# lukashermann/hulc

Hardware: AMD Instinct MI355X
Metric: trajectory-windows/sec (seq_len=32, bs=64/GPU) (higher is better)
Workload: dtype bf16; 1 GPU; HULC training step, vision goal only (use_clip_auxiliary_loss=false), B=64 windows/GPU, seq_len=32, 200x200 static + 84x84 gripper fp32 NCHW frames, fwd+loss+bwd+Adam, dropout 0.1; global_batch=64, seq_len=32, parallelism=dp1

## Files before the change

### hulc_amd/csrc/engine_backward.inc

```
    struct Bucket { int64_t lo, hi; };
    Bucket group_range(const char* prefix) const {
        int64_t lo = numel, hi = 0;
        const std::string a(prefix);
        for (size_t i = 0; i < tab_order.size(); ++i) {
            const auto& kv = tab_order[i];
            if (kv.first.compare(0, a.size(), a) == 0) { lo = std::min(lo, kv.second.off); hi = std::max(hi, i + 1 < tab_order.size() ? tab_order[i + 1].second.off : numel); }
        }
        if (hi <= lo) return Bucket{0, 0};
        return Bucket{lo, std::min<int64_t>(hi, numel)};
    }
    std::vector<std::pair<std::string, Ref>> tab_order;
    std::vector<Bucket> bucket_plan() const {
        std::vector<Bucket> v;
        const Bucket dec = group_range("action_decoder.");
        v.push_back(Bucket{dec.lo, numel});
        v.push_back(group_range("plan_proposal."));
        v.push_back(group_range("plan_recognition."));
        const Bucket vg = group_range("visual_goal."), lg = group_range("language_goal.");
        v.push_back(Bucket{std::min(vg.lo, lg.lo), std::max(vg.hi, lg.hi)});
        v.push_back(group_range("perceptual_encoder."));
        return v;
    }
    int comm_buckets(int64_t* lo, int64_t* hi, int cap) override {
        if (!bound) { hulc_set_error("hulc_comm_buckets before hulc_bind_params"); return -1; }
// ... 215 lines not shown
            }
            }
            if (mlp) {
                lin_wgrad(dH1, H1, HID, SB, HID, HID, mlp2.dW, HID, mlp2.db);
                { EpiP ep = epi(dZ1, false); ep.mask = H1; lin_dgrad(dH1, SB, mlp2, ep, dense_out(HID)); }
                lin_wgrad(dZ1, H0, HID, SB, HID, HID, mlp1.dW, HID, mlp1.db);
                { EpiP ep = epi(dZ0, false); ep.mask = H0; lin_dgrad(dZ1, SB, mlp1, ep, dense_out(HID)); }
                const int mp = ldpad(SB);
                transpose_pair(dZ0, HID, tA, SB, HID, embg, DE, tB, SB, DE, mp, cs16 ? dbih0 : nullptr, nullptr);
                h0t_valid = false;
                { EpiP ep = epi(dwih0 + dec_plan, true); ep.accumulate = 1; gemm(dense<T>(tA, HID, mp), dense<T>(tB, DE, mp), dense_out(KIN), ep, HID, DE, SB); }
            } else {
            rnn_bwd(dH1, H1, dZ1, whh1, B, S, 1, false, false, true);
            {
                const int mp = ldpad(SB);
                const bool fuse_cs = cs16;
                bool h0t_kept = false;
                if constexpr (std::is_same<T, h16_t>::value) {
                    if (!tB2) tB2 = alloc<T>(tcap);
                    if (tB2) { transpose_triple(dZ1, HID, tA, SB, HID, H1, HID, tB, SB, HID, H0, HID, tB2, SB, HID, mp, fuse_cs ? dbih1 : nullptr, fuse_cs ? dbhh1 : nullptr); h0t_kept = true; }
                }
                if (!h0t_kept)
                transpose_pair(dZ1, HID, tA, SB, HID, H1, HID, tB, SB, HID, mp, fuse_cs ? dbih1 : nullptr, fuse_cs ? dbhh1 : nullptr);
                h0t_valid = h0t_kept;
                if (S > 1) { EpiP ep = epi(whh1.dW, true); ep.accumulate = grad_first(whh1.dW) ? 0 : 1;
                  gemm(dense<T>(tA + B, HID, mp), dense<T>(tB, HID, mp), dense_out(HID), ep, HID, HID, (S - 1) * B); }
                if (!h0t_kept) cast_tr<T, T>(H0, HID, nullptr, 0, tB, mp, SB, HID);
                { EpiP ep = epi(wih1.dW, true); ep.accumulate = grad_first(wih1.dW) ? 0 : 1; gemm(dense<T>(tA, HID, mp), dense<T>(h0t_kept ? tB2 : tB, HID, mp), dense_out(HID), ep, HID, HID, SB); }
                if (!fuse_cs) colsum(dZ1, HID, SB, HID, dbih1, dbhh1);
            }
            { EpiP ep = epi(dH0, false); ep.out2 = dZ0 + lastBH; ep.out2_lo = lastBH; ep.out2_hi = lastBH + BH; ep.out2_mask = H0 + lastBH;
              gemm(dense<T>(dZ1, SB, HID), dense<T>(wih1.Wt, HID, HID), dense_out(HID), ep, SB, HID, HID); }
            rnn_bwd(dH0, H0, dZ0, whh0, B, S, 1, false, false, true);
            {
                const int mp = ldpad(SB);
                if (h0t_valid) {
                    transpose_pair(dZ0, HID, tA, SB, HID, embg, DE, tB, SB, DE, mp, cs16 ? dbih0 : nullptr, cs16 ? dbhh0 : nullptr);
                    if (S > 1) { EpiP ep = epi(whh0.dW, true); ep.accumulate = grad_first(whh0.dW) ? 0 : 1;
                      gemm(dense<T>(tA + B, HID, mp), dense<T>(tB2, HID, mp), dense_out(HID), ep, HID, HID, (S - 1) * B); }
                } else {
                transpose_pair(dZ0, HID, tA, SB, HID, H0, HID, tB, SB, HID, mp, cs16 ? dbih0 : nullptr, cs16 ? dbhh0 : nullptr);
                if (S > 1) { EpiP ep = epi(whh0.dW, true); ep.accumulate = grad_first(whh0.dW) ? 0 : 1;
                  gemm(dense<T>(tA + B, HID, mp), dense<T>(tB, HID, mp), dense_out(HID), ep, HID, HID, (S - 1) * B); }
                cast_tr<T, T>(embg, DE, nullptr, 0, tB, mp, SB, DE);
                }
                { EpiP ep = epi(dwih0 + dec_plan, true); ep.accumulate = 1; gemm(dense<T>(tA, HID, mp), dense<T>(tB, DE, mp), dense_out(KIN), ep, HID, DE, SB); }
            }
            }
            if (!bwd_skip_enc) { EpiP ep = epi(demb + (EMB - DE), true); ep.accumulate = 1;
              gemm(dense<T>(dZ0, SB, HID), dense<T>(wih0T + (long long)dec_plan * HID, DE, HID), dense_out_map(B, EMB, (long long)S * EMB), ep, SB, DE, HID); }
            hipLaunchKernelGGL((sum_over_t_kernel<T>), dim3(cdiv(BH, 256)), dim3(256), 0, st, dZ0, S, BH, dC);
            if constexpr (!std::is_same<T, h16_t>::value) colsum(dC, HID, B, HID, dbih0, dbhh0);
            else if (!cs16) colsum(dZ0, HID, SB, HID, dbih0, dbhh0);
            { EpiP ep = epi(dgoal, true); ep.accumulate = 1;
              gemm(dense<T>(dC, B, HID), dense<T>(wih0T + (long long)(dec_plan + DE) * HID, GOAL, HID), dense_out(GOAL), ep, B, GOAL, HID); }
            {
                const int mp = ldpad(B);
                transpose_pair(dC, HID, tA, B, HID, goal_t, GOAL, tB, B, GOAL, mp);
                EpiP ep = epi(dwih0 + dec_plan + DE, true); ep.accumulate = 1;
                gemm(dense<T>(tA, HID, mp), dense<T>(tB, GOAL, mp), dense_out(KIN), ep, HID, GOAL, B);
            }
            if (hulc) {
                { EpiP ep = epi(dplan, true); gemm(dense<T>(dC, B, HID), dense<T>(wih0T, PLAN, HID), dense_out(PLAN), ep, B, PLAN, HID); }
                launch_plan_scatter_grad<T>(st, plan_scatter_w4<T>(NCLS), dC, pidx, B, NCAT, NCLS, HID, KIN, dwih0, grads_fresh ? 1 : 0);
            }
            if (mcil) {
                { EpiP ep = epi(dplan, true); gemm(dense<T>(dC, B, HID), dense<T>(wih0T, dec_plan, HID), dense_out(dec_plan), ep, B, dec_plan, HID); }
                lin_wgrad(dC, plan_t, dec_plan, B, HID, dec_plan, dwih0, KIN, nullptr);
            }
        }
        const bool hold_buckets = hold_buckets_mode && mcil && !gru && ar_dtype >= 0 && persist_mode && !persist_under_comm && !(rp_probed && !rp_ok);
        if (!hold_buckets && bucket_ready(0)) return 1;
        if (hulc) {
            launch_st_softmax_bwd<T>(st, probs, dplan, dpr_kl, dpp_kl, B * NCAT, NCLS, dprl, dprl_t, dppl_t);
            DenseOut om = dense_out(EMB + GOAL);
            mlp_bwd(dppl_t, ppx, EMB + GOAL, B, pp, 5, ppa, dt_a, dt_a + (long long)B * HID, dppx, &om, 0);
            hipLaunchKernelGGL(pp_input_bwd_kernel, dim3(cdiv(B * (EMB + GOAL), 256)), dim3(256), 0, st, dppx, B, EMB, GOAL, demb, (long long)S * EMB, dgoal);
            if (bucket_ready(1)) return 1;
            if (wq_small(B)) wq_add(dprl_t, seqf_t, B, pr_fs);
            else lin_wgrad(dprl_t, seqf_t, FCH, B, PLAN, FCH, pr_fs.dW, FCH, pr_fs.db);
            { EpiP ep = epi(dseqf, true);
              if (have_dseq) ep.accumulate = 1;
              else { ep.out2 = dseq_t; ep.out2_lo = 0; ep.out2_hi = (long long)B * FCH; dseq_cast_done = true; }
              lin_dgrad(dprl_t, B, pr_fs, ep, dense_out(FCH)); }
            have_dseq = true;
        }
        if (mcil) {
            const int n = PLAN / 2;
            launch_normal_rsample_bwd<T>(st, dplan, plan_eps, pr_logits, dpr_kl, B, n, dprl_t);
            hipLaunchKernelGGL((cast_kernel<float, T>), dim3(cdiv(B * PLAN, 256)), dim3(256), 0, st, dpp_kl, dppl_t, (long long)B * PLAN);
            DenseOut om = dense_out(EMB + GOAL);
            mlp_bwd(dppl_t, ppx, EMB + GOAL, B, pp, 5, ppa, dt_a, dt_a + (long long)B * HID, dppx, &om, 0);
            hipLaunchKernelGGL(pp_input_bwd_kernel, dim3(cdiv(B * (EMB + GOAL), 256)), dim3(256), 0, st, dppx, B, EMB, GOAL, demb, (long long)S * EMB, dgoal);
            if (!hold_buckets && bucket_ready(1)) return 1;
            if (gru) bigru_bwd(dprl_t, B, S); else birnn_bwd(dprl_t, B, S);
            if (hold_buckets && (bucket_ready(0) || bucket_ready(1))) return 1;
        }
        if (have_dseq) {
            if (!dseq_cast_done) hipLaunchKernelGGL((cast_kernel<float, T>), dim3(cdiv(B * FCH, 256)), dim3(256), 0, st, dseqf, dseq_t, (long long)B * FCH);
            if (wq_small(B)) wq_add(dseq_t, xm, B, pr_fc);
            else lin_wgrad(dseq_t, xm, EMB, B, FCH, EMB, pr_fc.dW, EMB, pr_fc.db);
            { EpiP ep = epi(dxm, true); lin_dgrad(dseq_t, B, pr_fc, ep, dense_out(EMB)); }
            float* dx = dxa; float* dnext = dxb;
            if (!ln_bwd_can_bcast) hipLaunchKernelGGL(bcast_over_s_kernel, dim3(cdiv((long long)N * EMB, 256)), dim3(256), 0, st, dxm, B, S, EMB, dx);
            for (int l = 1; l >= 0; --l) {
                const bool bc = ln_bwd_can_bcast && l == 1;
                bool ffn_fused = false;
                if constexpr (std::is_same<T, h16_t>::value) ffn_fused = trf_on() && S <= 64;
                T *b_c = dt_c, *b_a = dt_a, *b_d = dt_c, *b_b = dt_b;
                bool defer_w = false;
                if constexpr (std::is_same<T, h16_t>::value) {
                    defer_w = ffn_fused;
                    if (defer_w) {
                        if (!trb_c[l]) { trb_c[l] = alloc<T>((int64_t)maxN * EMB); trb_a[l] = alloc<T>((int64_t)maxN * FF); trb_d[l] = alloc<T>((int64_t)maxN * EMB, l ? "tr_bd1" : "tr_bd0"); trb_b[l] = alloc<T>((int64_t)maxN * 3 * EMB, l ? "tr_bb1" : "tr_bb0"); }
                        b_c = trb_c[l]; b_a = trb_a[l]; b_d = trb_d[l]; b_b = trb_b[l];
                    }
// ... 41 lines not shown
                else lin_wgrad(b_d, ao[l], EMB, N, EMB, EMB, tr_out[l].dW, EMB, tr_out[l].db);
                { EpiP ep = epi(dt_a, false); lin_dgrad(b_d, N, tr_out[l], ep, dense_out(EMB)); }
                launch_attention_bwd<T>(st, attention_s64(S), qkv[l], Pat[l], dt_a, B, S, EMB, NH, b_b, dp, site_seed(1 + 4 * l));
                if (defer_w) wq_add(b_b, xt[l], N, tr_in[l]);
                else lin_wgrad(b_b, xt[l], EMB, N, 3 * EMB, EMB, tr_in[l].dW, EMB, tr_in[l].db);
                { EpiP ep = epi(dx, true); ep.res = dy_f; ep.res_f32 = 1; ep.res_ld = EMB; lin_dgrad(b_b, N, tr_in[l], ep, dense_out(EMB)); }
            }
            {
                const int bchunk = (std::is_same<T, float>::value || repro) ? B : 8;
                if (cdiv(B, bchunk) > 1) nd(ND_POS_EMB);
                hipLaunchKernelGGL(pr_input_bwd_kernel, dim3(cdiv(S * EMB, 256), cdiv(B, bchunk)), dim3(256), 0, st, dx, B, S, EMB, dp, site_seed(0), demb, dpos, bchunk);
            }
        }
        if (bucket_ready(1) || bucket_ready(2)) return 1;
        if (pair) {
            const int Bv = pairBv, Bl = B - pairBv;
            T* av[2] = {gl1, gl2};
            T* al[2] = {gl1 + (long long)Bv * HID, gl2 + (long long)Bv * HID};
            ln_bwd(dgoal, GOAL, gl3, GOAL, goal_st, ln_vg_g, Bv, GOAL, nullptr, 0, 0, dgl3_t, GOAL, d_ln_vg_g, d_ln_vg_b);
            DenseOut om = dense_out((long long)S * EMB);
            mlp_bwd(dgl3_t, emb + (long long)(S - 1) * EMB, (long long)S * EMB, Bv, vg, 3, av, dt_a, dt_a + (long long)B * HID, bwd_skip_enc ? nullptr : demb + (long long)(S - 1) * EMB, bwd_skip_enc ? nullptr : &om, bwd_skip_enc ? 0 : 1);
            ln_bwd(dgoal + Bv * GOAL, GOAL, gl3 + Bv * GOAL, GOAL, goal_st + 2 * Bv, ln_lg_g, Bl, GOAL, nullptr, 0, 0, dgl3_t + Bv * GOAL, GOAL, d_ln_lg_g, d_ln_lg_b);
            mlp_bwd(dgl3_t + Bv * GOAL, lang_t, LANG, Bl, lg, 3, al, dt_a, dt_a + (long long)B * HID, nullptr, nullptr, 0);
        } else {
            T* acts[2] = {gl1, gl2};
            if (b->is_lang) {
                ln_bwd(dgoal, GOAL, gl3, GOAL, goal_st, ln_lg_g, B, GOAL, nullptr, 0, 0, dgl3_t, GOAL, d_ln_lg_g, d_ln_lg_b);
                mlp_bwd(dgl3_t, lang_t, LANG, B, lg, 3, acts, dt_a, dt_a + (long long)B * HID, nullptr, nullptr, 0);
            } else {
                ln_bwd(dgoal, GOAL, gl3, GOAL, goal_st, ln_vg_g, B, GOAL, nullptr, 0, 0, dgl3_t, GOAL, d_ln_vg_g, d_ln_vg_b);
                DenseOut om = dense_out((long long)S * EMB);
                mlp_bwd(dgl3_t, emb + (long long)(S - 1) * EMB, (long long)S * EMB, B, vg, 3, acts, dt_a, dt_a + (long long)B * HID,
                        bwd_skip_enc ? nullptr : demb + (long long)(S - 1) * EMB, bwd_skip_enc ? nullptr : &om, bwd_skip_enc ? 0 : 1);
            }
        }
        }
        wq_flush();
        if (bucket_ready(3)) return 1;
        if (part == 0) {
            lazy_sweep(0, numel, st);
            if (hipGetLastError() != hipSuccess) { hulc_set_error("kernel launch failed in backward"); return 1; }
            bwd_stage = 1;
            return 0;
        }
        if (bwd_skip_enc) goto finish;
    encoders:
        {
            const Conv1Src src[2] = {conv1_src(*b, false), conv1_src(*b, true)}, src2[2] = {conv1_src(cur2, false), conv1_src(cur2, true)};
            const int Nenc = enc_frames(N);
            const bool tail_fused = enc_tail_fusable() && (!repro || enc_tail_bwd_room(Nenc));
            if (ragged()) launch_rows_reduce(st, demb, rg_lens(), rg_off(), B, S, EMB, demb_c);
            if (tail_fused) enc_tail_bwd_both(Nenc);
            enc_bwd_both(src, pair ? src2 : nullptr, Nenc, tail_fused);
            flush_unpacks();
        }
    finish:
        if (bucket_ready(4)) return 1;
        lazy_sweep(0, numel, st);
        if (hipGetLastError() != hipSuccess) { hulc_set_error("kernel launch failed in backward"); return 1; }
        have_fwd = false;
        bwd_stage = 0;
        grads_fresh = false;
        return 0;
    }
```

### hulc_amd/csrc/engine_encoders.inc

```
    ConvGeom geom(int Nf, int IH, int C, int K, int S) const {
        ConvGeom g; g.Nf = Nf; g.IH = g.IW = IH; g.C = C; g.KH = g.KW = K; g.S = S; g.OH = g.OW = (IH - K) / S + 1; return g;
    }
    Conv1Src conv1_src(const hulc_batch& b, bool gripper) const {
        Conv1Src s;
        s.X = gripper ? b.rgb_gripper : b.rgb_static;
        s.u8 = b.frames_u8 != 0;
        s.shift = s.u8 ? (gripper ? b.shift_gripper : b.shift_static) : nullptr;
        s.pad = gripper ? b.pad_gripper : b.pad_static;
        s.fold = (s.u8 && std::is_same<T, h16_t>::value && u8_fold_mode) ? 1 : 0;
        if (s.u8 && b.window_start) { s.wstart = reinterpret_cast<const long long*>(b.window_start); s.S = b.S; s.nstore = b.store_frames; }
        if (s.wstart && (b.window_len || b.window_len_host)) {
            const int set = &b == &cur2 ? 1 : 0;
            s.wstart = wl_frame[set]; s.S = 1;
            if (s.shift) s.shift = wl_shift[set][gripper ? 1 : 0];
        }
        return s;
    }
    static Conv1Src conv1_src_f32(const void* x) { return Conv1Src{x, nullptr, 0, 0}; }
    long long* wl_frame[2] = {nullptr, nullptr};
    int* wl_shift[2][2] = {{nullptr, nullptr}, {nullptr, nullptr}};
    int wl_alloc(int set) {
        if (!wl_frame[set]) {
            wl_frame[set] = alloc<long long>((int64_t)maxN); wl_shift[set][0] = alloc<int>((int64_t)maxN * 2); wl_shift[set][1] = alloc<int>((int64_t)maxN * 2);
            if (alloc_failed) { hulc_set_error("window_len: workspace allocation failed"); return 1; }
// ... 158 lines not shown
            const Stage S = stage(0, sn, Nf), G = stage(1, sn, Nf);
            const ConvTileP j[2] = {conv_fwd_job(S), conv_fwd_job(G)};
            TimerScope ts(this, "conv_tile_fwd", "mfma", 0, 0, 0);
            const bool ok = sn == 2 ? launch_conv_reg_fwd_jobs<32, 4, 4, 2>(st, j, 2) : launch_conv_reg_fwd_jobs<64, 3, 3, 1>(st, j, 2);
            if (ok) ts.add(conv_fwd_flops(S.c, S.g) + conv_fwd_flops(G.c, G.g), conv_fwd_bytes(S.c, S.g) + conv_fwd_bytes(G.c, G.g));
            return ok;
        }
        return false;
    }
    void enc_fwd_stages(int k0, int k1, const Conv1Src* src, const Conv1Src* src2, int Nf, bool defer_tail) {
        const bool both = k1 - k0 == 2;
        for (int k = k0; k < k1; ++k) conv1_fwd(k, src[k], Nf, src2 ? &src2[k] : nullptr);
        for (int sn = 2; sn <= 3; ++sn)
            if (!(both && conv_fwd_both(sn, Nf))) for (int k = k0; k < k1; ++k) conv_fwd(k, sn, Nf);
        for (int k = k0; k < k1; ++k) head_fwd(k, Nf, defer_tail);
    }
    void enc_fwd_both(const Conv1Src* src, const Conv1Src* src2, int Nf, bool defer_tail) {
        if constexpr (std::is_same<T, h16_t>::value) enc_fwd_stages(0, 2, src, src2, Nf, defer_tail);
        else for (int k = 0; k < 2; ++k) enc_fwd_stages(k, k + 1, src, src2, Nf, defer_tail);
    }
    bool enc_tail_fusable() const {
        if constexpr (!std::is_same<T, h16_t>::value) return false;
        auto ok = [](const EncW& e) { return e.fc1.K == 128 && e.fc1.N == 512 && e.fc2.K == 512 && e.fc2.N == 64; };
        return ok(encS) && ok(encG) && EMB == 128;
    }
    bool x0_done = false;
    void enc_tail_fwd_both(int Nf, bool with_x0 = false, int S = 1, float dp = 0.f) {
        if constexpr (std::is_same<T, h16_t>::value) {
            EncTailP q{};
            if (with_x0) { q.pos = pos32; q.xf = xf[0]; q.xt = xt[0]; q.z0 = y2[0]; q.z1 = y2[1]; q.S = S; q.drop_p = dp; q.seed = site_seed(0); x0_done = true; }
            for (int k = 0; k < 2; ++k) {
                const EncW& e = encw(k); EncA& a = enca(k);
                EncTailCam& c = q.cam[k];
                c.x = e.gripper ? a.g0 : a.ss; c.W1 = e.fc1.W; c.W2 = e.fc2.W; c.b1 = e.fc1.b32; c.b2 = e.fc2.b32;
                c.lng = e.lng; c.lnb = e.lnb; c.f1 = a.f1; c.f2 = a.f2; c.lnst = a.lnst; c.col0 = k * 64;
            }
            q.emb = enc_emb(); q.Nf = Nf; q.ldemb = EMB;
            launch_enc_tail_fwd(st, q);
        }
    }
    UnpackBatch unpack_jobs{};
    int64_t part_cur = 0;
    int unpack_blocks = 0;
    bool unpack_room(int jobs, int64_t floats) const { return unpack_jobs.n + jobs <= UNPACK_MAX_JOBS && part_cur + floats <= this->partcap; }
    float* queue_unpack(float* grad, int O, int I, int KH, int KW, int nhwc, int nsplit, int ysplit) {
        const long long slab = (long long)O * I * KH * KW;
        if (!unpack_room(1, nsplit * slab)) return nullptr;
        float* const slabs = this->part + part_cur;
        UnpackJob& U = unpack_jobs.j[unpack_jobs.n++];
        U.part = slabs; U.grad = grad; U.slab = slab; U.nsplit = nsplit; U.O = O; U.I = I; U.KH = KH; U.KW = KW; U.nhwc = nhwc; U.blk0 = unpack_blocks; U.ysplit = ysplit;
        unpack_blocks += cdiv((int)slab, 1024); part_cur += nsplit * slab;
        return slabs;
    }
    void flush_unpacks() {
        constexpr int yparts = 8;
        if (repro) for (int i = 0; i < unpack_jobs.n; ++i) unpack_jobs.j[i].ysplit = 1;
        else for (int i = 0; i < unpack_jobs.n; ++i) if (unpack_jobs.j[i].ysplit == 0 && unpack_jobs.j[i].nsplit > 1) nd(ND_CONV_UNPACK_SPLIT);
        if (unpack_jobs.n > 0) hipLaunchKernelGGL(unpack_conv_wgrad_batched_kernel, dim3(unpack_blocks, repro ? 1 : yparts), dim3(256), 0, st, unpack_jobs);
        unpack_jobs.n = 0; part_cur = 0; unpack_blocks = 0;
    }
    bool tail_fc7_done = false;
    void enc_tail_bwd_both(int Nf) {
        if constexpr (std::is_same<T, h16_t>::value) {
            EncTailBwdP q{};
            for (int k = 0; k < 2; ++k) {
                const EncW& e = encw(k); EncA& a = enca(k);
                EncTailBwdCam& c = q.cam[k];
                c.f2 = a.f2; c.lnst = a.lnst; c.lng = e.lng; c.f1 = a.f1; c.W2t = e.fc2.Wt; c.W1t = e.fc1.Wt;
                c.xmask = a.g0; c.dlng = e.dlng; c.dlnb = e.dlnb;
                c.d_f2 = a.d_f2t; c.d_f1 = a.d_f1; c.dx_f32 = a.d_ss; c.dx_t = a.d_g0; c.col0 = k * 64;
            }
            q.demb = enc_demb(); q.Nf = Nf; q.ldemb = EMB;
            const int nblk = cdiv(Nf, 16);
            const bool slab_pg = repro && nblk > 1;
            if (slab_pg) for (int k = 0; k < 2; ++k) q.cam[k].pg_slab = cspart + (long long)k * 2 * nblk * 64;
            if (!repro && Nf > 16) nd(ND_ENC_TAIL_LN);
            launch_enc_tail_bwd(st, q);
            if (slab_pg)
                for (int k = 0; k < 2; ++k) {
                    hipLaunchKernelGGL(colsum_final_kernel, dim3(1), dim3(256), 0, st, (const float*)q.cam[k].pg_slab, nblk, 64, encw(k).dlng, (float*)nullptr, 1.f);
                    hipLaunchKernelGGL(colsum_final_kernel, dim3(1), dim3(256), 0, st, (const float*)q.cam[k].pg_slab + (long long)nblk * 64, nblk, 64, encw(k).dlnb, (float*)nullptr, 1.f);
                }
            const int nz = enc_tail_nsplit(Nf);
            if (!repro && nz > 1) nd(ND_LIN_BWD_ROWS);
            LinStreamBatch bt{};
            int blk = 0;
            const bool cs_bias = repro && nz > 1;
            auto add = [&](const T* dY, const T* X, const LinW& L, float* dW, float* slabs) {
                lin_stream_add(bt, blk, (const h16_t*)dY, (const h16_t*)X, L.K, Nf, L.N, L.K, dW, L.K, cs_bias ? nullptr : L.db, slabs, nz, 0);
            };
            for (int k = 0; k < 2; ++k) {
                const EncW& e = encw(k); EncA& a = enca(k);
                add(a.d_f2t, a.f1, e.fc2, e.fc2.dW, queue_unpack(e.fc2.dW, e.fc2.N, e.fc2.K, 1, 1, 0, nz, 1));
                add(a.d_f1, e.gripper ? a.g0 : a.ss, e.fc1, e.fc1.dW, queue_unpack(e.fc1.dW, e.fc1.N, e.fc1.K, 1, 1, 0, nz, 1));
            }
            const LinW& L = encG.fc7;
            float* const slabs7 = L.N == 128 && L.K == 3136 ? queue_unpack(L.dW, 128, 64, 7, 7, 1, nz, 1) : nullptr;
            tail_fc7_done = slabs7 != nullptr;
            if (slabs7) add(aG.d_g0, aG.a3, L, nullptr, slabs7);
            launch_lin_stream(st, bt, blk);
            if (cs_bias) {
                for (int k = 0; k < 2; ++k) {
                    const EncW& e = encw(k); EncA& a = enca(k);
                    colsum(a.d_f2t, e.fc2.N, Nf, e.fc2.N, e.fc2.db);
                    colsum(a.d_f1, e.fc1.N, Nf, e.fc1.N, e.fc1.db);
                }
                if (slabs7) colsum(aG.d_g0, L.N, Nf, L.N, L.db);
            }
        }
    }
    static int enc_tail_nsplit(int Nf) { return lin_stream_nsplit(2 * (1 * 4 + 8 * 1) + 2 * 25, Nf); }
// ... 235 lines not shown
```

### hulc_amd/csrc/gemm.h

```cpp
#pragma once
#include "common.h"

namespace HULC_NS {

struct EpiP {
    void* out = nullptr;
    int out_f32 = 0;
    int accumulate = 0;
    int atomic = 0;
    long long z_stride = 0;
    const float* bias = nullptr;
    const float* bias2 = nullptr;
    const void* res = nullptr;
    int res_f32 = 0;
    long long res_ld = 0;
    int res_rowmod = 0;
    int res_late = 0;
    const void* mask = nullptr;
    int mask_tanh = 0;
    int relu = 0;
    float alpha = 1.f;
    float drop_p = 0.f;
    unsigned long long drop_seed = 0;
    void* out2 = nullptr;
// ... 747 lines not shown
#pragma unroll
    for (int mt = 0; mt < MT; ++mt)
#pragma unroll
        for (int r = 0; r < 4; ++r) red[wave][(mt * 4 + r) * 64 + lane] = acc[mt][r];
    __syncthreads();
    for (int idx = tid; idx < MT * 256; idx += NW * 64) {
        float v = 0.f;
#pragma unroll
        for (int w = 0; w < NW; ++w) v += red[w][idx];
        const int mt = idx >> 8, r = (idx >> 6) & 3, l = idx & 63;
        const int row = m0 + mt * 16 + (l >> 4) * 4 + r;
        const int col = n0 + (l & 15);
        if (row < M && col < N) {
            const int rrow = ep.res_rowmod > 0 ? row % ep.res_rowmod : row;
            epi_store<h16_t>(ep, v, rrow, col, om.offset(row, 0) + col);
        }
    }
}
#ifdef HULC_KERNEL_STAMPS
__device__ unsigned long long g_stamps[512 * 64];
#define KSTAMP(n) do { if (lane == 0) g_stamps[(blockIdx.y * gridDim.x + blockIdx.x) * 64 + wave * 8 + (n)] = __builtin_amdgcn_s_memtime(); } while (0)
#else
#define KSTAMP(n)
#endif
constexpr int FRAG_PACK_MAX = 24;
struct FragPackBatch { const h16_t* src[FRAG_PACK_MAX]; h16_t* dst[FRAG_PACK_MAX]; int N[FRAG_PACK_MAX], K[FRAG_PACK_MAX]; int blk0[FRAG_PACK_MAX + 1]; int n; };
static inline int frag_pack_blocks(int N, int K) { return (N / 16) * (K / ((K % 256) == 0 ? 256 : 128)); }
__global__ void __launch_bounds__(256) frag_pack_kernel(FragPackBatch b) {
    __shared__ uint4 tile[16][33];
    int j = 0;
    while (j + 1 < b.n && (int)blockIdx.x >= b.blk0[j + 1]) ++j;
    const int K = b.K[j], KT = (K % 256) == 0 ? 256 : 128, CPR = KT >> 3;
    const int kt_n = K / KT, blk = (int)blockIdx.x - b.blk0[j], nb = blk / kt_n, kt = blk % kt_n, t = threadIdx.x;
    const h16_t* __restrict__ src = b.src[j];
    h16_t* __restrict__ dst = b.dst[j];
#pragma unroll
    for (int r = 0; r < 2; ++r) {
        const int idx = t + 256 * r, row = idx / CPR, ch = idx % CPR;
        if (idx < 16 * CPR) tile[row][ch] = *reinterpret_cast<const uint4*>(src + (long long)(nb * 16 + row) * K + kt * KT + ch * 8);
    }
    __syncthreads();
#pragma unroll
    for (int r = 0; r < 2; ++r) {
        const int idx = t + 256 * r, ksl = idx >> 6, lane = idx & 63, g = lane >> 4, i = lane & 15;
        if (idx < 16 * CPR) *reinterpret_cast<uint4*>(dst + (((long long)nb * (K >> 5) + kt * (KT >> 5) + ksl) * 64 + lane) * 8) = tile[i][ksl * 4 + g];
    }
}
DEVI const h16_t* wfrag_ptr(const h16_t* Wf, int row0, int K, int k0, int lane) { return Wf + (((long long)(row0 >> 4) * (K >> 5) + (k0 >> 5)) * 64 + lane) * 8; }
DEVI const h16_t* skinny_wfrag_ptr(const h16_t* W, long long ldw, int n0, int Nclamp, int K, int kb, int lane, int* wstep) {
    if (ldw == 0) { *wstep = 512; return W + ((long long)(n0 >> 4) * (K >> 5) + (kb >> 5)) * 512 + lane * 8; }
    *wstep = 32;
    return W + (long long)min(n0 + (lane & 15), Nclamp) * ldw + kb + (lane >> 4) * 8;
}
struct Skinny2 { const h16_t* A; const h16_t* W; EpiP ep; };
template <int MT, int KQ32, int NW = 8, bool DUAL = false>
__global__ void __launch_bounds__(NW * 64) skinny_lds_kernel(const h16_t* __restrict__ A_, long long lda, const h16_t* __restrict__ W_,
                                                         long long ldw, int M, int N, int K, DenseOut om, EpiP ep_, Skinny2 p2 = Skinny2{}) {
    const bool second = DUAL && blockIdx.z != 0;
    const h16_t* __restrict__ A = second ? p2.A : A_;
    const h16_t* __restrict__ W = second ? p2.W : W_;
    const EpiP& ep = second ? p2.ep : ep_;
    constexpr int PCW = KQ32 / 2;
    extern __shared__ __attribute__((aligned(16))) char sk_smem[];
    typedef __attribute__((address_space(3))) char lchar;
    const int tid = threadIdx.x, lane = tid & 63, wave = tid >> 6;
    const int n0 = blockIdx.x * 16;
    const int m0 = blockIdx.y * (MT * 16);
    const int kq = KQ32 * 32, kb = wave * kq;
    const int g = lane >> 4, i = lane & 15;
    lchar* wbase = (lchar*)sk_smem + wave * (MT * 2 * PCW * 1024);
    KSTAMP(0);
    {
        const int r = lane >> 3, c = (lane & 7) ^ (r & 6);
#pragma unroll
        for (int rg = 0; rg < MT * 2; ++rg) {
            const h16_t* src = A + (long long)min(m0 + rg * 8 + r, M - 1) * lda + kb + c * 8;
#pragma unroll
            for (int pc = 0; pc < PCW; ++pc)
                lds_dma16(src + pc * 64, (unsigned)(size_t)(wbase + (rg * PCW + pc) * 1024));
        }
    }
    const h16_t* wp = W + (long long)min(n0 + i, N - 1) * ldw + kb + g * 8;
    h16x8_t b[KQ32];
#pragma unroll
    for (int u = 0; u < KQ32; ++u) b[u] = *reinterpret_cast<const h16x8_t*>(wp + u * 32);
    const int erow = m0 + (tid >> 6) * 16 + i, ecol = n0 + g * 4;
    const bool ethread = tid < MT * 64 && erow < M;
    const int errow = ep.res_rowmod > 0 ? erow % ep.res_rowmod : erow;
    const long long eo = ethread ? om.offset(erow, 0) + ecol : 0;
    const bool fast16 = epi_is_fast16(ep) && ecol + 3 < N && (eo & 3) == 0;
    EpiPre4 pre;
    EpiF16Pre fpre;
    if (ethread) { if (fast16) fpre = epi_fast16_pre(ep, errow, ecol, eo); else pre = epi_prefetch4<h16_t>(ep, errow, ecol, N, eo); }
    f32x4 acc[MT];
#pragma unroll
    for (int mt = 0; mt < MT; ++mt) acc[mt] = f32x4{0.f, 0.f, 0.f, 0.f};
    KSTAMP(1);
    asm volatile("s_waitcnt vmcnt(0)" ::: "memory");
    KSTAMP(2);
    {
        const int r = i & 7;
        lchar* fb = wbase + (i >> 3) * (PCW * 1024) + r * 128;
#pragma unroll
        for (int u = 0; u < KQ32; ++u) {
            const int chunk = ((u & 1) * 4 + g) ^ (r & 6);
#pragma unroll
            for (int mt = 0; mt < MT; ++mt) {
                const h16x8_t a = *(__attribute__((address_space(3))) h16x8_t*)(fb + (mt * 2 * PCW + (u >> 1)) * 1024 + chunk * 16);
                acc[mt] = MFMA_16x16x32_H(b[u], a, acc[mt], 0, 0, 0);
            }
        }
    }
    KSTAMP(3);
    __syncthreads();
    KSTAMP(4);
    f32x4* red = reinterpret_cast<f32x4*>(sk_smem);
#pragma unroll
    for (int mt = 0; mt < MT; ++mt) red[(wave * MT + mt) * 64 + lane] = acc[mt];
    __syncthreads();
// ... 252 lines not shown
    if (K % 2048 != 0 || K <= 2048 || M > 64 || (lda % 64) != 0 || ((uintptr_t)A % 128) != 0 || (N % 16) != 0) return false;
    return !(A2 && ((uintptr_t)A2 % 128) != 0);
}
static inline bool launch_skinny_lds_kchunk(hipStream_t st, const h16_t* A, long long lda, const h16_t* W, long long ldw, int M, int N, int K, const DenseOut& om,
                                            const EpiP& ep, const GruBwdP& gb = GruBwdP{}, const KChunk2* p2 = nullptr) {
    if (!skinny_lds_kchunk_ok(A, lda, M, N, K, p2 ? p2->A : nullptr)) return false;
    max_dyn_lds_once<&skinny_lds_kchunk_kernel<2, 4, 16>>(160 * 1024);
    hipLaunchKernelGGL((skinny_lds_kchunk_kernel<2, 4, 16>), dim3(N / 16, (M + 31) / 32, p2 ? 2 : 1), dim3(1024), (size_t)16 * 2 * 2 * 2 * 1024, st, A, lda, W, ldw, M, N, K, om, ep, gb,
                       p2 ? *p2 : KChunk2{});
    return true;
}

template <int MT, int KQ32>
static inline void launch_skinny_lds_t(hipStream_t st, dim3 grid, const h16_t* A, long long lda, const h16_t* W, long long ldw, int M, int N, int K,
                                       const DenseOut& om, const EpiP& ep) {
    const size_t lds = (size_t)8 * MT * 2 * (KQ32 / 2) * 1024;
    max_dyn_lds_once<&skinny_lds_kernel<MT, KQ32>>(160 * 1024);
    hipLaunchKernelGGL((skinny_lds_kernel<MT, KQ32>), grid, dim3(512), lds, st, A, lda, W, ldw, M, N, K, om, ep);
}
static inline bool launch_skinny_lds(hipStream_t st, const h16_t* A, long long lda, const h16_t* W, long long ldw, int M, int N, int K, int MT,
                                     const DenseOut& om, const EpiP& ep) {
    if (K % 512 != 0 || K > 2048 || (lda % 64) != 0 || ((uintptr_t)A % 128) != 0) return false;
    if ((size_t)MT * 16 * K * 2 > 128 * 1024 || (MT != 2 && MT != 4 && !(MT == 1 && K == 2048))) return false;
    dim3 grid(N / 16, (M + MT * 16 - 1) / (MT * 16));
    const int kq32 = K / 256;
#define SKL(mt, kq) launch_skinny_lds_t<mt, kq>(st, grid, A, lda, W, ldw, M, N, K, om, ep)
    if (MT == 1) {
        max_dyn_lds_once<&skinny_lds_kernel<1, 4, 16>>(160 * 1024);
        hipLaunchKernelGGL((skinny_lds_kernel<1, 4, 16>), grid, dim3(1024), (size_t)16 * 1 * 2 * 2 * 1024, st, A, lda, W, ldw, M, N, K, om, ep);
        return true;
    }
    if (MT == 2 && kq32 == 8) {
        max_dyn_lds_once<&skinny_lds_kernel<2, 4, 16>>(160 * 1024);
        hipLaunchKernelGGL((skinny_lds_kernel<2, 4, 16>), grid, dim3(1024), (size_t)16 * 2 * 2 * 2 * 1024, st, A, lda, W, ldw, M, N, K, om, ep);
        return true;
    }
    if (MT == 2) { if (kq32 == 4) SKL(2, 4); else if (kq32 == 2) SKL(2, 2); else return false; }
    else { if (kq32 == 4) SKL(4, 4); else if (kq32 == 2) SKL(4, 2); else return false; }
#undef SKL
    return true;
}
static inline bool skinny_lds_dual_ok(const h16_t* A0, const h16_t* W0, const h16_t* A1, const h16_t* W1, long long lda, long long ldw, int M, int N, int K) {
    return !(K != 2048 || M <= 32 || M > 64 || (N % 16) != 0 || (lda % 64) != 0 || ((uintptr_t)A0 % 128) != 0 || ((uintptr_t)A1 % 128) != 0 ||
             ((uintptr_t)W0 % 16) != 0 || ((uintptr_t)W1 % 16) != 0 || (ldw % 8) != 0);
}
static inline bool launch_skinny_lds_dual(hipStream_t st, const h16_t* A0, const h16_t* W0, const EpiP& ep0, const h16_t* A1, const h16_t* W1, const EpiP& ep1, long long lda,
                                          long long ldw, int M, int N, int K, const DenseOut& om) {
    if (!skinny_lds_dual_ok(A0, W0, A1, W1, lda, ldw, M, N, K)) return false;
    max_dyn_lds_once<&skinny_lds_kernel<2, 4, 16, true>>(160 * 1024);
    Skinny2 p2; p2.A = A1; p2.W = W1; p2.ep = ep1;
    hipLaunchKernelGGL((skinny_lds_kernel<2, 4, 16, true>), dim3(N / 16, (M + 31) / 32, 2), dim3(1024), (size_t)16 * 2 * 2 * 2 * 1024, st, A0, lda, W0, ldw, M, N, K, om, ep0, p2);
    return true;
}
template <int NW>
static inline void launch_skinny_nw(hipStream_t st, const h16_t* A, long long lda, const h16_t* W, long long ldw, int M, int N, int K,
                                    const DenseOut& om, const EpiP& ep, bool use_lds = true) {
    int MT = M >= 64 ? 4 : (M + 15) / 16;
    if (M > 32 && (N / 16) * ((M + 63) / 64) <= 160) MT = 2;
    if (M > 32 && K == 2048 && NW == 8) MT = 2;
    if (M > 16 && M <= 32 && K == 2048 && NW == 8 && (N / 16) * 2 <= 320) MT = 1;
    if (NW == 8 && use_lds && launch_skinny_lds(st, A, lda, W, ldw, M, N, K, MT, om, ep)) return;
    dim3 grid(N / 16, (M + MT * 16 - 1) / (MT * 16)), block(NW * 64);
    switch (MT) {
        case 1: hipLaunchKernelGGL((skinny_gemm_kernel<NW, 1>), grid, block, 0, st, A, lda, W, ldw, M, N, K, om, ep); break;
        case 2: hipLaunchKernelGGL((skinny_gemm_kernel<NW, 2>), grid, block, 0, st, A, lda, W, ldw, M, N, K, om, ep); break;
        case 3: hipLaunchKernelGGL((skinny_gemm_kernel<NW, 3>), grid, block, 0, st, A, lda, W, ldw, M, N, K, om, ep); break;
        default: hipLaunchKernelGGL((skinny_gemm_kernel<NW, 4>), grid, block, 0, st, A, lda, W, ldw, M, N, K, om, ep); break;
    }
}
static inline void launch_skinny(hipStream_t st, const h16_t* A, long long lda, const h16_t* W, long long ldw, int M, int N, int K,
                                 const DenseOut& om, const EpiP& ep, bool use_lds = true) {
    if (use_lds && M > 16 && launch_skinny_lds_kchunk(st, A, lda, W, ldw, M, N, K, om, ep)) return;
    if (K % 512 == 0) launch_skinny_nw<8>(st, A, lda, W, ldw, M, N, K, om, ep, use_lds);
    else launch_skinny_nw<4>(st, A, lda, W, ldw, M, N, K, om, ep, use_lds);
}
static inline bool skinny_ok(int M, int N, int K, long long lda, long long ldw, const void* A, const void* W) {
    const bool shape = M <= 64 || (K >= 512 && (long long)M * N <= 524288 && (long long)((M + 63) / 64) * (N / 16) >= 16);
    return shape && (K % 32) == 0 && K >= 128 && (N % 16) == 0 && (lda % 8) == 0 && (ldw % 8) == 0 && ((uintptr_t)A % 16) == 0 && ((uintptr_t)W % 16) == 0;
}

enum GemmPick { GEMM_PICK_SKINNY = 0, GEMM_PICK_GLDS, GEMM_PICK_128_BK64, GEMM_PICK_128_BK32, GEMM_PICK_64_BK128, GEMM_PICK_64_BK32, GEMM_PICK_32_BK128, GEMM_PICK_32_BK32 };
static inline int gemm_pick_tile(GemmPick p) {
    switch (p) {
        case GEMM_PICK_SKINNY: return 0;
        case GEMM_PICK_GLDS: case GEMM_PICK_128_BK64: case GEMM_PICK_128_BK32: return 128;
        case GEMM_PICK_64_BK128: case GEMM_PICK_64_BK32: return 64;
        default: return 32;
    }
}
template <typename T>
static inline GemmPick gemm_pick(const DenseLoader<T>& a, const DenseLoader<T>& b, const EpiP& ep, int M, int N, int K) {
    constexpr bool H16 = sizeof(T) == 2;
    if constexpr (H16) {
        if (a.R1 == 0x7fffffff && b.R1 == 0x7fffffff && ep.z_stride == 0 && skinny_ok(M, N, K, a.s1, b.s1, a.p, b.p)) return GEMM_PICK_SKINNY;
    }
    const long long w128 = (long long)((M + 127) / 128) * ((N + 127) / 128), w64 = (long long)((M + 63) / 64) * ((N + 63) / 64);
    if (M >= 512 && N >= 128 && w128 >= 128) {
        if constexpr (H16) {
            if (gemm_glds_ok(a, b, ep, M, N, K)) return GEMM_PICK_GLDS;
            if (K >= 128) return GEMM_PICK_128_BK64;
        }
        return GEMM_PICK_128_BK32;
    }
    const bool t64 = w64 >= 128 || (M <= 64 && N <= 64);
    if (H16 && K >= 128) return t64 ? GEMM_PICK_64_BK128 : GEMM_PICK_32_BK128;
    return t64 ? GEMM_PICK_64_BK32 : GEMM_PICK_32_BK32;
// ... 34 lines not shown
```

### hulc_amd/csrc/kernels.h

```cpp
#pragma once
#include "common.h"

namespace HULC_NS {

template <typename TS, typename TD>
__global__ void __launch_bounds__(256) cast_transpose_kernel(const TS* __restrict__ src, long long lds_, TD* __restrict__ dst,
                                                             long long ldd, TD* __restrict__ dstT, long long ldt, int R, int C) {
    __shared__ float tile[32][33];
    const int c0 = blockIdx.x * 32, r0 = blockIdx.y * 32;
    const int tx = threadIdx.x & 31, ty = threadIdx.x >> 5;
#pragma unroll
    for (int i = 0; i < 4; ++i) {
        const int r = r0 + ty + i * 8, c = c0 + tx;
        float v = 0.f;
        if (r < R && c < C) {
            v = to_f<TS>(src[(long long)r * lds_ + c]);
            if (dst) dst[(long long)r * ldd + c] = from_f<TD>(v);
        }
        tile[ty + i * 8][tx] = v;
    }
    if (!dstT) return;
    __syncthreads();
#pragma unroll
    for (int i = 0; i < 4; ++i) {
// ... 132 lines not shown
        const int r = r0 + ty + i * 8, c = c0 + tx;
        tile[ty + i * 8][tx] = (r < D.R && c < D.C) ? to_f<T>(src[(long long)r * D.lds + c]) : 0.f;
    }
    __syncthreads();
#pragma unroll
    for (int i = 0; i < 4; ++i) {
        const int c = c0 + ty + i * 8, r = r0 + tx;
        if (r < D.R && c < D.C) dst[(long long)c * D.ldt + r] = from_f<T>(tile[tx][ty + i * 8]);
    }
}

struct ConvPackBatch { const float* w[6]; void* wf[6]; void* wd[6]; int O[6], I[6], K[6], S[6], nhwc[6], blk0[7]; };

__global__ void unpack_conv_wgrad_kernel(const float* __restrict__ part, int nsplit, long long slab, float* __restrict__ grad,
                                         int O, int I, int KH, int KW, int nhwc_fwd) {
    const int idx = (blockIdx.x * blockDim.x + threadIdx.x) * 4;
    const int total = O * I * KH * KW;
    if (idx >= total) return;
    const int per = (nsplit + gridDim.y - 1) / gridDim.y;
    const int z0 = blockIdx.y * per, z1 = min(nsplit, z0 + per);
    float4 s0 = make_float4(0.f, 0.f, 0.f, 0.f), s1 = s0, s2 = s0, s3 = s0;
    auto add4 = [](float4& a, const float4 b) { a.x += b.x; a.y += b.y; a.z += b.z; a.w += b.w; };
    int z = z0;
    for (; z + 7 < z1; z += 8) {
        float4 t[8];
#pragma unroll
        for (int u = 0; u < 8; ++u) t[u] = *reinterpret_cast<const float4*>(part + (long long)(z + u) * slab + idx);
        add4(s0, t[0]); add4(s1, t[1]); add4(s2, t[2]); add4(s3, t[3]);
        add4(s0, t[4]); add4(s1, t[5]); add4(s2, t[6]); add4(s3, t[7]);
    }
    for (; z + 3 < z1; z += 4) {
        const float4 a = *reinterpret_cast<const float4*>(part + (long long)z * slab + idx), b = *reinterpret_cast<const float4*>(part + (long long)(z + 1) * slab + idx);
        const float4 c = *reinterpret_cast<const float4*>(part + (long long)(z + 2) * slab + idx), d = *reinterpret_cast<const float4*>(part + (long long)(z + 3) * slab + idx);
        add4(s0, a); add4(s1, b); add4(s2, c); add4(s3, d);
    }
    for (; z < z1; ++z) add4(s0, *reinterpret_cast<const float4*>(part + (long long)z * slab + idx));
    const float v[4] = {(s0.x + s1.x) + (s2.x + s3.x), (s0.y + s1.y) + (s2.y + s3.y), (s0.z + s1.z) + (s2.z + s3.z), (s0.w + s1.w) + (s2.w + s3.w)};
#pragma unroll
    for (int e = 0; e < 4; ++e) {
        int dst = idx + e;
        if (nhwc_fwd) {
            int ci = dst % I, t = dst / I;
            int kw = t % KW; t /= KW;
            int kh = t % KH, o = t / KH;
            dst = ((o * I + ci) * KH + kh) * KW + kw;
        }
        if (gridDim.y > 1) unsafeAtomicAdd(grad + dst, v[e]);
        else grad[dst] += v[e];
    }
}

struct UnpackJob { const float* part; float* grad; long long slab; int nsplit, O, I, KH, KW, nhwc, blk0, ysplit; };
constexpr int UNPACK_MAX_JOBS = 12;
struct UnpackBatch { UnpackJob j[UNPACK_MAX_JOBS]; int n; };
__global__ void unpack_conv_wgrad_batched_kernel(UnpackBatch ub) {
    int k = 0;
    while (k + 1 < ub.n && (int)blockIdx.x >= ub.j[k + 1].blk0) ++k;
    const UnpackJob J = ub.j[k];
    const int idx = ((blockIdx.x - J.blk0) * blockDim.x + threadIdx.x) * 4;
    const int total = J.O * J.I * J.KH * J.KW;
    if (idx >= total) return;
    const int gy = J.ysplit > 0 ? J.ysplit : (int)gridDim.y;
    if ((int)blockIdx.y >= gy) return;
    const int per = (J.nsplit + gy - 1) / gy;
    const int z0 = blockIdx.y * per, z1 = min(J.nsplit, z0 + per);
    if (z0 >= z1) return;
    const float* part = J.part;
    const long long slab = J.slab;
    float4 s0 = make_float4(0.f, 0.f, 0.f, 0.f), s1 = s0, s2 = s0, s3 = s0;
    auto add4 = [](float4& a, const float4 b) { a.x += b.x; a.y += b.y; a.z += b.z; a.w += b.w; };
    int z = z0;
    for (; z + 7 < z1; z += 8) {
        float4 t[8];
#pragma unroll
        for (int u = 0; u < 8; ++u) t[u] = *reinterpret_cast<const float4*>(part + (long long)(z + u) * slab + idx);
        add4(s0, t[0]); add4(s1, t[1]); add4(s2, t[2]); add4(s3, t[3]);
        add4(s0, t[4]); add4(s1, t[5]); add4(s2, t[6]); add4(s3, t[7]);
    }
    for (; z + 3 < z1; z += 4) {
        const float4 a = *reinterpret_cast<const float4*>(part + (long long)z * slab + idx), b = *reinterpret_cast<const float4*>(part + (long long)(z + 1) * slab + idx);
        const float4 c = *reinterpret_cast<const float4*>(part + (long long)(z + 2) * slab + idx), d = *reinterpret_cast<const float4*>(part + (long long)(z + 3) * slab + idx);
        add4(s0, a); add4(s1, b); add4(s2, c); add4(s3, d);
    }
    for (; z < z1; ++z) add4(s0, *reinterpret_cast<const float4*>(part + (long long)z * slab + idx));
    const float v[4] = {(s0.x + s1.x) + (s2.x + s3.x), (s0.y + s1.y) + (s2.y + s3.y), (s0.z + s1.z) + (s2.z + s3.z), (s0.w + s1.w) + (s2.w + s3.w)};
    if (gy == 1 && !J.nhwc) {
        float4* g4 = reinterpret_cast<float4*>(J.grad + idx);
        float4 o = *g4;
        o.x += v[0]; o.y += v[1]; o.z += v[2]; o.w += v[3];
        *g4 = o;
        return;
    }
#pragma unroll
    for (int e = 0; e < 4; ++e) {
        int dst = idx + e;
        if (J.nhwc) {
            int ci = dst % J.I, t = dst / J.I;
            int kw = t % J.KW; t /= J.KW;
            int kh = t % J.KH, o = t / J.KH;
            dst = ((o * J.I + ci) * J.KH + kh) * J.KW + kw;
        }
        if (gy == 1) J.grad[dst] += v[e];
        else unsafeAtomicAdd(J.grad + dst, v[e]);
    }
}

template <typename TS, typename TD>
__global__ void permute_cols_kernel(const TS* __restrict__ src, TD* __restrict__ dst, int R, int CH, int P, int inverse,
// ... 2382 lines not shown
```

Measured before the change: 21830 windows/s.

## Fuse dplan/dgoal skinny GEMMs and fold stale-grad zeroing into unpack kernel

Adds a segmented skinny LDS GEMM that computes the dplan and dgoal input-gradient GEMMs, which share the dC operand, in one launch. It also routes the goal weight-gradient through the small-batch wgrad queue when applicable. Zeroing of stale lazy gradient regions is folded into the batched conv-wgrad unpack kernel as extra blocks, so a separate lazy sweep has less to do when no allreduce runs. The aim is fewer kernel launches and fewer passes over dC, at the cost of more kernel complexity and a zeroing path that only applies under certain conditions.

```diff
diff --git a/hulc_amd/csrc/engine_backward.inc b/hulc_amd/csrc/engine_backward.inc
--- a/hulc_amd/csrc/engine_backward.inc
+++ b/hulc_amd/csrc/engine_backward.inc
@@ -291,16 +291,29 @@
             hipLaunchKernelGGL((sum_over_t_kernel<T>), dim3(cdiv(BH, 256)), dim3(256), 0, st, dZ0, S, BH, dC);
             if constexpr (!std::is_same<T, h16_t>::value) colsum(dC, HID, B, HID, dbih0, dbhh0);
             else if (!cs16) colsum(dZ0, HID, SB, HID, dbih0, dbhh0);
-            { EpiP ep = epi(dgoal, true); ep.accumulate = 1;
-              gemm(dense<T>(dC, B, HID), dense<T>(wih0T + (long long)(dec_plan + DE) * HID, GOAL, HID), dense_out(GOAL), ep, B, GOAL, HID); }
-            {
+            bool dplan_done = false;
+            { EpiP eg = epi(dgoal, true); eg.accumulate = 1;
+              const T* const wgoal = wih0T + (long long)(dec_plan + DE) * HID;
+              if constexpr (std::is_same<T, h16_t>::value) {
+                  if (hulc) {
+                      const EpiP epl = epi(dplan, true);
+                      if (gemm_pick<T>(dense<T>(dC, B, HID), dense<T>(wih0T, PLAN, HID), epl, B, PLAN, HID) == GEMM_PICK_SKINNY &&
+                          gemm_pick<T>(dense<T>(dC, B, HID), dense<T>(wgoal, GOAL, HID), eg, B, GOAL, HID) == GEMM_PICK_SKINNY) {
+                          TimerScope ts(this, "skinny_gemm_m64", "hbm", 2.0 * B * (PLAN + GOAL) * HID, ((double)B * HID + (double)(PLAN + GOAL) * HID + (double)B * (PLAN + GOAL)) * sizeof(T));
+                          dplan_done = launch_skinny_lds_seg2(st, dC, HID, wih0T, wgoal, HID, B, PLAN, GOAL, HID, dense_out(PLAN), epl, dense_out(GOAL), eg);
+                      }
+                  }
+              }
+              if (!dplan_done) gemm(dense<T>(dC, B, HID), dense<T>(wgoal, GOAL, HID), dense_out(GOAL), eg, B, GOAL, HID); }
+            if (wq_small(B)) wq_add(dC, goal_t, GOAL, B, HID, GOAL, dwih0 + dec_plan + DE, KIN, nullptr);
+            else {
                 const int mp = ldpad(B);
                 transpose_pair(dC, HID, tA, B, HID, goal_t, GOAL, tB, B, GOAL, mp);
                 EpiP ep = epi(dwih0 + dec_plan + DE, true); ep.accumulate = 1;
                 gemm(dense<T>(tA, HID, mp), dense<T>(tB, GOAL, mp), dense_out(KIN), ep, HID, GOAL, B);
             }
             if (hulc) {
-                { EpiP ep = epi(dplan, true); gemm(dense<T>(dC, B, HID), dense<T>(wih0T, PLAN, HID), dense_out(PLAN), ep, B, PLAN, HID); }
+                if (!dplan_done) { EpiP ep = epi(dplan, true); gemm(dense<T>(dC, B, HID), dense<T>(wih0T, PLAN, HID), dense_out(PLAN), ep, B, PLAN, HID); }
                 launch_plan_scatter_grad<T>(st, plan_scatter_w4<T>(NCLS), dC, pidx, B, NCAT, NCLS, HID, KIN, dwih0, grads_fresh ? 1 : 0);
             }
             if (mcil) {
@@ -448,7 +461,7 @@
             if (ragged()) launch_rows_reduce(st, demb, rg_lens(), rg_off(), B, S, EMB, demb_c);
             if (tail_fused) enc_tail_bwd_both(Nenc);
             enc_bwd_both(src, pair ? src2 : nullptr, Nenc, tail_fused);
-            flush_unpacks();
+            flush_unpacks(ar_dtype < 0);
         }
     finish:
         if (bucket_ready(4)) return 1;
diff --git a/hulc_amd/csrc/engine_encoders.inc b/hulc_amd/csrc/engine_encoders.inc
--- a/hulc_amd/csrc/engine_encoders.inc
+++ b/hulc_amd/csrc/engine_encoders.inc
@@ -234,11 +234,23 @@
         unpack_blocks += cdiv((int)slab, 1024); part_cur += nsplit * slab;
         return slabs;
     }
-    void flush_unpacks() {
+    void flush_unpacks(bool sweep = false) {
         constexpr int yparts = 8;
         if (repro) for (int i = 0; i < unpack_jobs.n; ++i) unpack_jobs.j[i].ysplit = 1;
         else for (int i = 0; i < unpack_jobs.n; ++i) if (unpack_jobs.j[i].ysplit == 0 && unpack_jobs.j[i].nsplit > 1) nd(ND_CONV_UNPACK_SPLIT);
-        if (unpack_jobs.n > 0) hipLaunchKernelGGL(unpack_conv_wgrad_batched_kernel, dim3(unpack_blocks, repro ? 1 : yparts), dim3(256), 0, st, unpack_jobs);
+        const int gy = repro ? 1 : yparts;
+        int zblocks = 0;
+        unpack_jobs.zblk0 = -1; unpack_jobs.nz = 0;
+        if (sweep && unpack_jobs.n > 0) {
+            long long quads = 0;
+            for (LazyG& z : lazy)
+                if (z.stale && unpack_jobs.nz < UNPACK_MAX_ZERO) { unpack_jobs.zp[unpack_jobs.nz] = G + z.off; unpack_jobs.zn[unpack_jobs.nz] = z.n; ++unpack_jobs.nz; quads += z.n >> 2; z.stale = false; }
+            if (unpack_jobs.nz) {
+                zblocks = (int)std::max<long long>(1, std::min<long long>(cdiv(512, gy), cdiv(quads, 256ll * 8 * gy)));
+                unpack_jobs.zblk0 = unpack_blocks;
+            }
+        }
+        if (unpack_jobs.n > 0) hipLaunchKernelGGL(unpack_conv_wgrad_batched_kernel, dim3(unpack_blocks + zblocks, gy), dim3(256), 0, st, unpack_jobs);
         unpack_jobs.n = 0; part_cur = 0; unpack_blocks = 0;
     }
     bool tail_fc7_done = false;
diff --git a/hulc_amd/csrc/gemm.h b/hulc_amd/csrc/gemm.h
--- a/hulc_amd/csrc/gemm.h
+++ b/hulc_amd/csrc/gemm.h
@@ -823,19 +823,22 @@
     *wstep = 32;
     return W + (long long)min(n0 + (lane & 15), Nclamp) * ldw + kb + (lane >> 4) * 8;
 }
-struct Skinny2 { const h16_t* A; const h16_t* W; EpiP ep; };
-template <int MT, int KQ32, int NW = 8, bool DUAL = false>
+struct Skinny2 { const h16_t* A; const h16_t* W; EpiP ep; int blk0; int N; DenseOut om; };
+template <int MT, int KQ32, int NW = 8, bool DUAL = false, bool SEG = false>
 __global__ void __launch_bounds__(NW * 64) skinny_lds_kernel(const h16_t* __restrict__ A_, long long lda, const h16_t* __restrict__ W_,
-                                                         long long ldw, int M, int N, int K, DenseOut om, EpiP ep_, Skinny2 p2 = Skinny2{}) {
-    const bool second = DUAL && blockIdx.z != 0;
-    const h16_t* __restrict__ A = second ? p2.A : A_;
+                                                         long long ldw, int M, int N_, int K, DenseOut om_, EpiP ep_, Skinny2 p2 = Skinny2{}) {
+    const bool seg = SEG && (int)blockIdx.x >= p2.blk0;
+    const bool second = (DUAL && blockIdx.z != 0) || seg;
+    const h16_t* __restrict__ A = (second && !SEG) ? p2.A : A_;
     const h16_t* __restrict__ W = second ? p2.W : W_;
     const EpiP& ep = second ? p2.ep : ep_;
+    const int N = seg ? p2.N : N_;
+    const DenseOut& om = seg ? p2.om : om_;
     constexpr int PCW = KQ32 / 2;
     extern __shared__ __attribute__((aligned(16))) char sk_smem[];
     typedef __attribute__((address_space(3))) char lchar;
     const int tid = threadIdx.x, lane = tid & 63, wave = tid >> 6;
-    const int n0 = blockIdx.x * 16;
+    const int n0 = (seg ? (int)blockIdx.x - p2.blk0 : (int)blockIdx.x) * 16;
     const int m0 = blockIdx.y * (MT * 16);
     const int kq = KQ32 * 32, kb = wave * kq;
     const int g = lane >> 4, i = lane & 15;
@@ -1194,6 +1197,25 @@
     hipLaunchKernelGGL((skinny_lds_kernel<2, 4, 16, true>), dim3(N / 16, (M + 31) / 32, 2), dim3(1024), (size_t)16 * 2 * 2 * 2 * 1024, st, A0, lda, W0, ldw, M, N, K, om, ep0, p2);
     return true;
 }
+static inline bool skinny_lds_seg2_ok(const h16_t* A, long long lda, const h16_t* W0, const h16_t* W1, long long ldw, int M, int N0, int N1, int K) {
+    return K == 2048 && M >= 1 && M <= 64 && (N0 % 16) == 0 && (N1 % 16) == 0 && N0 / 16 * 2 <= 320 && N1 / 16 * 2 <= 320 && (lda % 64) == 0 && ((uintptr_t)A % 128) == 0 &&
+           ((uintptr_t)W0 % 16) == 0 && ((uintptr_t)W1 % 16) == 0 && (ldw % 8) == 0;
+}
+static inline bool launch_skinny_lds_seg2(hipStream_t st, const h16_t* A, long long lda, const h16_t* W0, const h16_t* W1, long long ldw, int M, int N0, int N1, int K,
+                                          const DenseOut& om0, const EpiP& ep0, const DenseOut& om1, const EpiP& ep1) {
+    if (!skinny_lds_seg2_ok(A, lda, W0, W1, ldw, M, N0, N1, K)) return false;
+    Skinny2 p2; p2.A = A; p2.W = W1; p2.ep = ep1; p2.blk0 = N0 / 16; p2.N = N1; p2.om = om1;
+    const int MT = M > 32 ? 2 : 1;
+    const dim3 grid((N0 + N1) / 16, (M + MT * 16 - 1) / (MT * 16));
+    if (MT == 2) {
+        max_dyn_lds_once<&skinny_lds_kernel<2, 4, 16, false, true>>(160 * 1024);
+        hipLaunchKernelGGL((skinny_lds_kernel<2, 4, 16, false, true>), grid, dim3(1024), (size_t)16 * 2 * 2 * 2 * 1024, st, A, lda, W0, ldw, M, N0, K, om0, ep0, p2);
+    } else {
+        max_dyn_lds_once<&skinny_lds_kernel<1, 4, 16, false, true>>(160 * 1024);
+        hipLaunchKernelGGL((skinny_lds_kernel<1, 4, 16, false, true>), grid, dim3(1024), (size_t)16 * 1 * 2 * 2 * 1024, st, A, lda, W0, ldw, M, N0, K, om0, ep0, p2);
+    }
+    return true;
+}
 template <int NW>
 static inline void launch_skinny_nw(hipStream_t st, const h16_t* A, long long lda, const h16_t* W, long long ldw, int M, int N, int K,
                                     const DenseOut& om, const EpiP& ep, bool use_lds = true) {
diff --git a/hulc_amd/csrc/kernels.h b/hulc_amd/csrc/kernels.h
--- a/hulc_amd/csrc/kernels.h
+++ b/hulc_amd/csrc/kernels.h
@@ -208,8 +208,20 @@
 
 struct UnpackJob { const float* part; float* grad; long long slab; int nsplit, O, I, KH, KW, nhwc, blk0, ysplit; };
 constexpr int UNPACK_MAX_JOBS = 12;
-struct UnpackBatch { UnpackJob j[UNPACK_MAX_JOBS]; int n; };
+constexpr int UNPACK_MAX_ZERO = 32;
+struct UnpackBatch { UnpackJob j[UNPACK_MAX_JOBS]; int n; int zblk0, nz; float* zp[UNPACK_MAX_ZERO]; long long zn[UNPACK_MAX_ZERO]; };
 __global__ void unpack_conv_wgrad_batched_kernel(UnpackBatch ub) {
+    if (ub.zblk0 >= 0 && (int)blockIdx.x >= ub.zblk0) {
+        const long long nzx = (long long)gridDim.x - ub.zblk0, stride = nzx * gridDim.y * blockDim.x;
+        const long long i0 = (((long long)blockIdx.x - ub.zblk0) + nzx * blockIdx.y) * blockDim.x + threadIdx.x;
+        const float4 z = {0.f, 0.f, 0.f, 0.f};
+        for (int r = 0; r < ub.nz; ++r) {
+            float4* __restrict__ d = reinterpret_cast<float4*>(ub.zp[r]);
+            const long long n4 = ub.zn[r] >> 2;
+            for (long long i = i0; i < n4; i += stride) d[i] = z;
+        }
+        return;
+    }
     int k = 0;
     while (k + 1 < ub.n && (int)blockIdx.x >= ub.j[k + 1].blk0) ++k;
     const UnpackJob J = ub.j[k];
```

Measured after the change: 21950 windows/s, median of 6. Within noise of the previous version (+0.5%).
